# menonsamir/spiral

Hardware: AMD Instinct MI355X
Metric: server ms/query + DB GB/s vs HBM roofline, 2^20 x 256B (lower is better)
Workload: dtype u32 residues, 32x32->64-bit integer MAC (two 28-bit CRT primes)

## Files before the change

include/spiral_gpu.h:

```cpp
#ifndef SPIRAL_GPU_H
#define SPIRAL_GPU_H

#include <stddef.h>
#include <stdint.h>

#ifdef __cplusplus
extern "C" {
#endif

#define SPIRAL_GPU_ABI_VERSION 1

typedef struct spiral_gpu_params {
    uint32_t nu1;
    uint32_t nu2;
    uint32_t t_gsw;
    uint32_t t_conv;
    uint32_t t_exp;
    uint32_t t_exp_right;
    uint32_t qprime_bits;
    uint32_t direct_upload;
    uint64_t p_db;
} spiral_gpu_params;

typedef struct spiral_gpu_shape {
    uint32_t dim0, num_per, ell, m2, g, stopround;
    uint32_t n_left;
    uint32_t n_right;
    uint32_t n_query_cts;
    uint32_t n_bits;
    uint64_t qprime;
} spiral_gpu_shape;

typedef struct spiral_gpu_server spiral_gpu_server;

int spiral_gpu_abi_version(void);
const char *spiral_gpu_last_error(void);
int spiral_gpu_device_count(void);
int spiral_gpu_get_shape(const spiral_gpu_params *p, spiral_gpu_shape *out);
int spiral_gpu_has_limb_form(const spiral_gpu_params *p, uint32_t j_begin, uint32_t j_end);
int spiral_gpu_column_shard_has_limb_form(const spiral_gpu_params *p, uint32_t n_ranks);

int spiral_gpu_set_option(const char *name, int64_t value);
int spiral_gpu_get_option(const char *name, int64_t *value);

int spiral_gpu_get_tables(uint64_t *out);
int spiral_gpu_ntt_forward(uint64_t *operand, size_t npolys);
int spiral_gpu_ntt_inverse(uint64_t *operand, size_t npolys);
int spiral_gpu_to_ntt(uint64_t *out, const uint64_t *in, size_t npolys, int reduce);
int spiral_gpu_from_ntt(uint64_t *out, const uint64_t *in, size_t npolys);
int spiral_gpu_time_ntt(size_t npolys, int iters, float *fwd_ms, float *inv_ms);
int spiral_gpu_time_ntt_digits(size_t npolys, uint32_t n_digits, int iters, float *ms);
int spiral_gpu_multiply(uint64_t *out, const uint64_t *a, const uint64_t *b, size_t rs, size_t ms, size_t cs);
int spiral_gpu_add(uint64_t *out, const uint64_t *a, const uint64_t *b, size_t npolys);
int spiral_gpu_mul_by_const(uint64_t *out, const uint64_t *single_poly, const uint64_t *a, size_t npolys);
int spiral_gpu_automorph(uint64_t *out, const uint64_t *in, size_t npolys, uint64_t t);
int spiral_gpu_invert(uint64_t *out, const uint64_t *in, size_t npolys);
int spiral_gpu_gadget_invert(uint64_t *out, const uint64_t *in, size_t mx, size_t rdim, size_t cols);
int spiral_gpu_get_rescaled(uint64_t *out, const uint64_t *in, size_t n, uint64_t inp_mod, uint64_t out_mod);

size_t spiral_gpu_response_wire_bytes(const spiral_gpu_params *p, uint32_t out_n);
int spiral_gpu_response_from_wire(const spiral_gpu_params *p, uint32_t out_n, const void *wire, uint64_t *response);

int spiral_gpu_multiply_query_by_database(uint64_t *output, const uint64_t *reorientedCiphertexts,
                                          const uint64_t *database, size_t dim0, size_t num_per);
int spiral_gpu_multiply_queries_by_database(uint64_t *outputs, const uint64_t *reorientedCiphertexts, size_t n,
                                            const uint64_t *database, size_t dim0, size_t num_per);
int spiral_gpu_split_and_crt(uint64_t *out, const uint64_t *in, size_t num_per, uint32_t t_gsw);
int spiral_gpu_fold_one_further_dimension(uint64_t *cts, size_t num_per, const uint64_t *query_ct,
// ... 251 lines not shown
```

spiral_amd/_lib.py:

```python
from __future__ import annotations

import ctypes as C
import os
import subprocess

import numpy as np

HERE = os.path.dirname(os.path.abspath(__file__))
LIB_PATH = os.environ.get("SPIRAL_LIB") or os.path.join(HERE, "libspiral_gpu.so")
CSRC = os.path.join(HERE, "csrc")


class Params(C.Structure):

    _fields_ = [
        ("nu1", C.c_uint32),
        ("nu2", C.c_uint32),
        ("t_gsw", C.c_uint32),
        ("t_conv", C.c_uint32),
        ("t_exp", C.c_uint32),
        ("t_exp_right", C.c_uint32),
        ("qprime_bits", C.c_uint32),
        ("direct_upload", C.c_uint32),
        ("p_db", C.c_uint64),
# ... 14 lines not shown
        ("n_bits", C.c_uint32),
        ("qprime", C.c_uint64),
    ]


class PackShape(C.Structure):
    _fields_ = [(n, C.c_uint32) for n in ("dim0", "num_per", "ell", "g", "stopround", "n_left", "n_right", "n_query_cts", "trials")] + [
        ("qprime", C.c_uint64)
    ]


U64P = C.POINTER(C.c_uint64)

PROTOTYPES = {
    "spiral_gpu_abi_version": (C.c_int, []),
    "spiral_gpu_last_error": (C.c_char_p, []),
    "spiral_gpu_device_count": (C.c_int, []),
    "spiral_gpu_get_shape": (C.c_int, [C.POINTER(Params), C.POINTER(Shape)]),
    "spiral_gpu_has_limb_form": (C.c_int, [C.POINTER(Params), C.c_uint32, C.c_uint32]),
    "spiral_gpu_column_shard_has_limb_form": (C.c_int, [C.POINTER(Params), C.c_uint32]),
    "spiral_gpu_set_option": (C.c_int, [C.c_char_p, C.c_int64]),
    "spiral_gpu_get_option": (C.c_int, [C.c_char_p, C.POINTER(C.c_int64)]),
    "spiral_gpu_get_tables": (C.c_int, [U64P]),
    "spiral_gpu_ntt_forward": (C.c_int, [U64P, C.c_size_t]),
    "spiral_gpu_ntt_inverse": (C.c_int, [U64P, C.c_size_t]),
    "spiral_gpu_to_ntt": (C.c_int, [U64P, U64P, C.c_size_t, C.c_int]),
    "spiral_gpu_from_ntt": (C.c_int, [U64P, U64P, C.c_size_t]),
    "spiral_gpu_time_ntt": (C.c_int, [C.c_size_t, C.c_int, C.POINTER(C.c_float), C.POINTER(C.c_float)]),
    "spiral_gpu_time_ntt_digits": (C.c_int, [C.c_size_t, C.c_uint32, C.c_int, C.POINTER(C.c_float)]),
    "spiral_gpu_multiply": (C.c_int, [U64P, U64P, U64P, C.c_size_t, C.c_size_t, C.c_size_t]),
    "spiral_gpu_add": (C.c_int, [U64P, U64P, U64P, C.c_size_t]),
    "spiral_gpu_mul_by_const": (C.c_int, [U64P, U64P, U64P, C.c_size_t]),
    "spiral_gpu_automorph": (C.c_int, [U64P, U64P, C.c_size_t, C.c_uint64]),
    "spiral_gpu_invert": (C.c_int, [U64P, U64P, C.c_size_t]),
    "spiral_gpu_gadget_invert": (C.c_int, [U64P, U64P, C.c_size_t, C.c_size_t, C.c_size_t]),
    "spiral_gpu_get_rescaled": (C.c_int, [U64P, U64P, C.c_size_t, C.c_uint64, C.c_uint64]),
    "spiral_gpu_multiply_query_by_database": (C.c_int, [U64P, U64P, U64P, C.c_size_t, C.c_size_t]),
    "spiral_gpu_multiply_queries_by_database": (C.c_int, [U64P, U64P, C.c_size_t, U64P, C.c_size_t, C.c_size_t]),
    "spiral_gpu_split_and_crt": (C.c_int, [U64P, U64P, C.c_size_t, C.c_uint32]),
    "spiral_gpu_fold_one_further_dimension": (C.c_int, [U64P, C.c_size_t, U64P, U64P, C.c_uint32]),
    "spiral_gpu_expand_improved": (C.c_int, [U64P, C.c_uint32, C.c_uint32, U64P, C.c_uint32, U64P, C.c_uint32, C.c_uint32, C.c_uint32]),
    "spiral_gpu_scal_to_mat": (C.c_int, [U64P, U64P, U64P, C.c_uint32]),
    "spiral_gpu_regev_to_gsw": (C.c_int, [U64P, U64P, U64P, U64P, C.c_uint32, C.c_uint32]),
    "spiral_gpu_server_create": (C.c_int, [C.POINTER(Params), C.c_int, C.c_uint32, C.c_uint32, C.POINTER(C.c_void_p)]),
    "spiral_gpu_server_create_column_shard": (C.c_int, [C.POINTER(Params), C.c_int, C.c_uint32, C.c_uint32, C.POINTER(C.c_void_p)]),
    "spiral_gpu_server_destroy": (None, [C.c_void_p]),
# ... 265 lines not shown
```

spiral_amd/csrc/digits_device.h:

```cpp
#pragma once
#include <type_traits>

#include "common.h"
#include "ntt_device.h"

namespace spiral {

__device__ __forceinline__ uint64_t splitmix64(uint64_t x) {
    x += 0x9E3779B97F4A7C15ull;
    x = (x ^ (x >> 30)) * 0xBF58476D1CE4E5B9ull;
    x = (x ^ (x >> 27)) * 0x94D049BB133111EBull;
    return x ^ (x >> 31);
}

__device__ __forceinline__ uint64_t load_raw(const uint64_t* src, uint32_t idx, uint32_t tinv) {
    if (tinv == 0) return src[idx];
    uint32_t e = (idx * tinv) & (2 * kN - 1);
    uint64_t v = src[e & (kN - 1)];
    return (e & kN) ? kQ - v : v;
}

__device__ __forceinline__ uint64_t digit_of(uint64_t v, uint32_t k, uint32_t bits, uint64_t mask) {
    uint32_t sh = k * bits;
    if (bits <= 27u) {
        const bool up = sh >= 32u;
        const uint32_t d = __builtin_amdgcn_alignbit(up ? 0u : hi32(v), up ? hi32(v) : lo32(v), sh & 31u) & (uint32_t)mask;
        return sh >= 64 ? 0u : d;
    }
    return sh >= 64 ? 0ull : ((v >> sh) & mask);
}

__device__ __forceinline__ void udigits8(const uint64_t* raw, uint32_t k, uint32_t bits, uint32_t* d) {
    const uint32_t sh = k * bits, mask = (1u << bits) - 1u;
    if (sh >= 64u) {
#pragma unroll
        for (int r = 0; r < 8; r++) d[r] = 0;
    } else if (sh >= 32u) {
#pragma unroll
        for (int r = 0; r < 8; r++) d[r] = (hi32(raw[r]) >> (sh - 32u)) & mask;
    } else {
#pragma unroll
        for (int r = 0; r < 8; r++) d[r] = __builtin_amdgcn_alignbit(hi32(raw[r]), lo32(raw[r]), sh) & mask;
    }
}
__device__ __forceinline__ uint32_t udiv_small(uint32_t b, uint32_t d, uint32_t inv) { return d == 1u ? b : __umulhi(b, inv); }

template <bool SMALL>
__device__ __forceinline__ uint32_t digit_residue(uint32_t d, uint32_t m) {
    if constexpr (SMALL) return d;
    return d < (1u << 28) ? d : d % m;
}
constexpr uint32_t kSmallDigitBits = 27;
#define DIGIT_WIDTH_DISPATCH(bits, body) \
    do {                                 \
        if ((bits) <= kSmallDigitBits)   \
            body(std::true_type{});      \
        else                             \
            body(std::false_type{});     \
    } while (0)

struct SDigit {
    uint32_t sh_chain, sh_digit;
    uint64_t low_mask, thresh_in;
    uint64_t mask, base, thresh;
    bool has_in, may;
// ... 156 lines not shown
```

spiral_amd/csrc/kernels.h:

```cpp
#pragma once
#include <hip/hip_runtime.h>
#include <stdint.h>
#include <stdlib.h>

#include <atomic>

#include "common.h"

namespace spiral {

struct IndexMap {
    uint32_t inner, outer_stride, off;
    __host__ __device__ uint32_t operator()(uint32_t b) const { return (b / inner) * outer_stride + (b % inner) + off; }
};
inline IndexMap identity_map() { return IndexMap{1u, 1u, 0u}; }

#ifdef SPIRAL_TUNING
inline const char* tuning_env(const char* name) { return getenv(name); }
#else
inline const char* tuning_env(const char*) { return nullptr; }
#endif
struct Options {
    int fold_pair = 1, fold_chain = 1, fwd2 = -1;
    uint32_t fold_blocks = 768, sweep_mfma_min = 2, fwd2_min = 8192;
    size_t db_stage_bytes = (size_t)64 << 20;
    int one_image = 1;
    uint32_t pack_item_group = 0;
    uint32_t pack_batch_lanes = 0;
    int pack_pair_blocks = 0;
    int sweep_narrow = 0;
    uint32_t query_batch_chunk = 512;
};
Options& options();

#ifndef SPIRAL_MAX_LANES
#define SPIRAL_MAX_LANES 8
#endif
constexpr uint32_t kMaxLanes = SPIRAL_MAX_LANES;
struct Lanes {
    uint32_t n = 1;
    int64_t off[kMaxLanes] = {};
#ifdef __HIPCC__
    __device__ __forceinline__ int64_t here() const {
        const uint32_t z = blockIdx.z;
        int64_t o = 0;
#pragma unroll
        for (uint32_t q = 1; q < kMaxLanes; q++) o = z == q ? off[q] : o;
// ... 15 lines not shown
    __device__ __forceinline__ int64_t at(int64_t) const { return 0; }
#endif
};
struct Slots {
    uint32_t n = 1;
    int64_t stride = 0;
#ifdef __HIPCC__
    __device__ __forceinline__ int64_t here() const { return (int64_t)blockIdx.z * stride; }
    __device__ __forceinline__ int64_t at(int64_t s) const { return (int64_t)blockIdx.z * s; }
#endif
};
template <class P>
inline typename P::NoLanesT no_lanes(const P& p) {
    typename P::NoLanesT q{};
    static_cast<typename P::Core&>(q) = static_cast<const typename P::Core&>(p);
    return q;
}

struct DeviceTables {
    uint4* fwd = nullptr;
    uint4* inv = nullptr;
    uint64_t* neg1 = nullptr;
    uint64_t* neg1s = nullptr;
};
int tables_get(int device, DeviceTables* out);
void tables_host_rows(uint64_t* out8x2048);

constexpr bool lazy_ok(uint32_t terms) { return (unsigned __int128)terms * (2ull * kP - 1ull) * (kP - 1ull) < ((unsigned __int128)1 << 64); }
static_assert(lazy_ok(56) && lazy_ok(2 * 56) && lazy_ok(128) && !lazy_ok(129), "u64 accumulators hold up to 128 lazy products");

enum FwdLoad : uint32_t {
    LD_RAW = 0,
    LD_DIGIT = 1,
    LD_SDIGIT = 2,
    LD_LIMBS = 3,
    LD_DBGEN = 4,
    LD_PDIGIT = 6,
    LD_DBGEN1 = 7,
    LD_SDIFF = 8,
    LD_PDIFF = 9,
    LD_EXPAND = 5,
    LD_WIRE = 10,
};
constexpr uint32_t kWireCoeffBytes = 7;
constexpr uint32_t kWirePolyBytes = kWireCoeffBytes * 2048u;
enum FwdStore : uint32_t {
    ST_PK = 0,
    ST_REF = 1,
    ST_DB = 2,
// ... 422 lines not shown
```

spiral_amd/csrc/ntt.hip:

```cpp
#include <algorithm>
#include <cstdio>
#include <cstdlib>
#include <type_traits>

#include "digits_device.h"
#include "kernels.h"
#include "ntt_device.h"
#include "wire_device.h"

namespace spiral {

__device__ __forceinline__ void pk_load8_red(const uint64_t* poly, bool reduce, uint32_t tid, uint32_t* lo, uint32_t* hi) {
    uint64_t x[8];
    pk_load8(poly, tid, x);
    pk_unpack8(x, lo, hi);
    if (reduce) {
#pragma unroll
        for (int r = 0; r < 8; r++) {
            lo[r] %= kP;
            hi[r] %= kB;
        }
    }
}

// ... 411 lines not shown
    auto body = [&](auto small) {
#pragma unroll
        for (int r = 0; r < 8; r++) {
            const uint32_t d0 = (uint32_t)digit_of(raw[r], k0, bits, mask), d1 = (uint32_t)digit_of(raw[r], k1, bits, mask);
            lo0[r] = digit_residue<decltype(small)::value>(d0, kP);
            hi0[r] = digit_residue<decltype(small)::value>(d0, kB);
            lo1[r] = digit_residue<decltype(small)::value>(d1, kP);
            hi1[r] = digit_residue<decltype(small)::value>(d1, kB);
        }
    };
    DIGIT_WIDTH_DISPATCH(bits, body);
    ntt_forward_block2<false>(lo0, hi0, lo1, hi1, sh[0], sh[1], t.fwd, tid);
    const bool lazy = LOAD == LD_EXPAND || p.lazy_out != 0;
    if (!lazy) {
        canonicalize8(lo0, hi0);
        canonicalize8(lo1, hi1);
    }
    uint64_t v[8];
    pk_pack8(lo0, hi0, v);
    pk_store8(p.dst + (size_t)p.dst_map(ob + k0) * kN, tid, v);
    if (two) {
        pk_pack8(lo1, hi1, v);
        pk_store8(p.dst + (size_t)p.dst_map(ob + k1) * kN, tid, v);
    }
}

template <uint32_t STORE, bool EXPAND, class L>
__global__ __launch_bounds__(256, 8) void ntt_inverse_kernel(Tables t, InvParamsT<L> p) {
    __shared__ uint64_t sh[kLdsWords];
    const uint32_t tid = threadIdx.x, b = blockIdx.x;
    {
        const int64_t lane = p.lanes.here();
        lane_shift(p.src, lane);
        lane_shift(p.dst, lane);
        if constexpr (EXPAND) {
            lane_shift(p.cv, lane);
            lane_shift(p.query, lane);
        }
    }
    uint32_t lo[8], hi[8];
    if constexpr (EXPAND) {
        const uint32_t a = b >> 1, row = b & 1u;
        const uint32_t i = p.act.index(a, p.cnt_e);
#ifdef EXP_ABL_NO_ROW1
        if (row == 1) return;
#endif
// ... 156 lines not shown
        else                                                                                                                             \
            hipLaunchKernelGGL((KERNEL<__VA_ARGS__, NoLanes>), dim3((GRIDX), 1, 1), dim3(256), 0, s, TB, no_lanes(P));                   \
    } while (0)
#define FWD_CASE(L, S)                                                   \
    if (load == L && store == S) {                                       \
        LAUNCH_LANES(ntt_forward_kernel, nblocks, tb, p, L, S);          \
        return;                                                          \
    }

void launch_ntt_forward(const DeviceTables& t, const FwdParams& p_in, uint32_t load, uint32_t store, uint32_t nblocks, hipStream_t s) {
    if (nblocks == 0) return;
    FwdParams p = p_in;
    auto inv = [](uint32_t d) { return d > 1u ? (uint32_t)((1ull << 32) / d + 1ull) : 0u; };
    p.inv_n_digits = inv(p.n_digits);
    p.inv_te = inv(p.t_e);
    p.inv_to = inv(p.t_o);
    Tables tb{t.fwd, t.inv};
    const int fwd2_opt = options().fwd2;
    const bool fwd2 = (fwd2_opt >= 0 ? fwd2_opt != 0 : (uint64_t)nblocks * p.lanes.n >= options().fwd2_min) && p.tinv == 0;
    if ((uint64_t)nblocks * std::max({p.n_digits, p.t_e, p.t_o, 1u}) >= (1ull << 32)) {
        fprintf(stderr, "launch_ntt_forward: %u jobs exceed the range of the job-index division\n", nblocks);
        abort();
    }
    if (fwd2 && store == ST_PK && load == LD_DIGIT && p.n_digits >= 2) {
        const uint32_t nsrc = nblocks / p.n_digits;
        LAUNCH_LANES(ntt_forward2_kernel, nsrc * ((p.n_digits + 1u) / 2u), tb, p, LD_DIGIT);
        return;
    }
    if (fwd2 && store == ST_PK && load == LD_SDIFF && p.n_digits >= 2) {
        const uint32_t nsrc = nblocks / p.n_digits;
        LAUNCH_LANES(ntt_forward2_kernel, nsrc * ((p.n_digits + 1u) / 2u), tb, p, LD_SDIFF);
        return;
    }
    if (fwd2 && store == ST_PK && load == LD_PDIFF && p.n_digits >= 2) {
        const uint32_t nsrc = nblocks / p.n_digits;
        LAUNCH_LANES(ntt_forward2_kernel, nsrc * ((p.n_digits + 1u) / 2u), tb, p, LD_PDIFF);
        return;
    }
    if (fwd2 && store == ST_PK && load == LD_EXPAND) {
        const uint32_t cnt_o = p.t_o ? (nblocks - p.cnt_e * p.t_e) / p.t_o : 0u;
        LAUNCH_LANES(ntt_forward2_kernel, p.cnt_e * ((p.t_e + 1u) / 2u) + cnt_o * ((p.t_o + 1u) / 2u), tb, p, LD_EXPAND);
        return;
    }
    FWD_CASE(LD_RAW, ST_PK)
    FWD_CASE(LD_RAW, ST_REF)
    FWD_CASE(LD_DIGIT, ST_PK)
// ... 51 lines not shown
```

spiral_amd/csrc/ntt_device.h:

```cpp
#pragma once
#include "common.h"
#ifndef TWI
#define TWI(i) (i)
#endif
struct TwTable {
    __amdgpu_buffer_rsrc_t rs;
    __device__ __forceinline__ explicit TwTable(const uint4* tw) : rs(__builtin_amdgcn_make_buffer_rsrc(const_cast<uint4*>(tw), 0, 2048 * 16, 0x00020000)) {}
    __device__ __forceinline__ uint4 operator[](uint32_t i) const {
        typedef unsigned int u32x4_t __attribute__((ext_vector_type(4)));
        const u32x4_t v = __builtin_amdgcn_raw_buffer_load_b128(rs, i * 16u, 0, 0);
        return make_uint4(v.x, v.y, v.z, v.w);
    }
};
#ifdef NTT_PRIO
#define NTT_PRIO_HI() __builtin_amdgcn_s_setprio(NTT_PRIO)
#define NTT_PRIO_LO() __builtin_amdgcn_s_setprio(0)
#else
#define NTT_PRIO_HI() ((void)0)
#define NTT_PRIO_LO() ((void)0)
#endif
#ifdef NTT_ABLATE_BARRIER
#define NTT_SYNC() ((void)0)
#else
#define NTT_SYNC() __syncthreads()
// ... 216 lines not shown
        else
            dst[q * 256] = x;
    }
}
__device__ __forceinline__ void pk_unpack8(const uint64_t (&v)[8], uint32_t* lo, uint32_t* hi) {
#pragma unroll
    for (int k = 0; k < 8; k++) {
        lo[k] = lo32(v[k]);
        hi[k] = hi32(v[k]);
    }
}
__device__ __forceinline__ void pk_pack8(const uint32_t* lo, const uint32_t* hi, uint64_t (&v)[8]) {
#pragma unroll
    for (int k = 0; k < 8; k++) v[k] = pack(lo[k], hi[k]);
}

__device__ __forceinline__ void canonicalize8(uint32_t* lo, uint32_t* hi) {
#pragma unroll
    for (int k = 0; k < 8; k++) {
        lo[k] = csub_min(lo[k], kP);
        hi[k] = csub_min(hi[k], kB);
    }
}
template <bool CANONICAL = true>
__device__ __forceinline__ void ntt_forward_block(uint32_t* lo, uint32_t* hi, uint64_t* sh, const uint4* tw, uint32_t tid) {
    const TwTable tb(tw);
    Tw7 wb = tw_load8(tb, 8 + (tid >> 5), 16 + 2 * (tid >> 5), 32 + 4 * (tid >> 5));
#ifndef NTT_ABLATE_AB
    ct_radix8(lo, hi, tw, 1, 2, 4);
#endif
    NTT_PRIO_HI();
    lds_put<ix_a>(sh, tid, lo, hi);
    NTT_SYNC();
    lds_get<ix_b>(sh, tid, lo, hi);
    Tw7 wc = tw_load8(tb, 64 + (tid >> 2), 128 + 2 * (tid >> 2), 256 + 4 * (tid >> 2));
    NTT_PRIO_LO();
#ifndef NTT_ABLATE_AB
    ct_radix8_pre(lo, hi, wb);
#endif
    NTT_PRIO_HI();
    lds_put<ix_b>(sh, tid, lo, hi);
    NTT_SYNC();
    lds_get<ix_c>(sh, tid, lo, hi);
    Tw7 wd = tw_load4x2(tb, 512 + 2 * tid, 1024 + 4 * tid);
    NTT_PRIO_LO();
#pragma unroll
    for (int k = 0; k < 4; k++) {
        lo[k] = lazy_reduce(lo[k], kP);
        hi[k] = lazy_reduce(hi[k], kB);
    }
    ct_radix8_pre(lo, hi, wc);
    NTT_PRIO_HI();
#ifndef NTT_ABLATE_QUAD_EXCHANGE
    lds_put<ix_c>(sh, tid, lo, hi);
    NTT_SYNC();
    lds_get<ix_d>(sh, tid, lo, hi);
#endif
    NTT_PRIO_LO();
    ct_radix4x2_pre(lo, hi, wd);
#pragma unroll
    for (int k = 0; k < 8; k++) {
        lo[k] = lazy_reduce(lo[k], kP);
        hi[k] = lazy_reduce(hi[k], kB);
        if constexpr (CANONICAL) {
            lo[k] = csub_min(lo[k], kP);
            hi[k] = csub_min(hi[k], kB);
        }
    }
}

template <bool CANONICAL = true>
__device__ __forceinline__ void ntt_inverse_block(uint32_t* lo, uint32_t* hi, uint64_t* sh, const uint4* tw, uint32_t tid) {
    const TwTable tb(tw);
    Tw7 wd = tw_load4x2(tb, 512 + 2 * tid, 1024 + 4 * tid);
    Tw7 wc = tw_load8(tb, 64 + (tid >> 2), 128 + 2 * (tid >> 2), 256 + 4 * (tid >> 2));
    gs_radix4x2_pre(lo, hi, wd);
    NTT_PRIO_HI();
#ifndef NTT_ABLATE_QUAD_EXCHANGE
    lds_put<ix_d>(sh, tid, lo, hi);
    __syncthreads();
    lds_get<ix_c>(sh, tid, lo, hi);
#endif
    Tw7 wb = tw_load8(tb, 8 + (tid >> 5), 16 + 2 * (tid >> 5), 32 + 4 * (tid >> 5));
    NTT_PRIO_LO();
    gs_radix8_pre(lo, hi, wc);
    NTT_PRIO_HI();
    lds_put<ix_c>(sh, tid, lo, hi);
    __syncthreads();
    lds_get<ix_b>(sh, tid, lo, hi);
// ... 86 lines not shown
```

spiral_amd/csrc/primitives.cpp:

```cpp
#include "server_state.h"

thread_local std::string spiral::host::g_err;
std::atomic<uint64_t> spiral::host::g_pack_lane_batches{0};
std::atomic<uint64_t> spiral::g_mfma_sweeps{0};
std::atomic<uint64_t> spiral::host::g_db_export_ns{0};

spiral::Options& spiral::options() {
    static Options o = [] {
        Options v;
        if (const char* e = getenv("SPIRAL_FOLD_PAIR")) v.fold_pair = atoi(e) != 0;
        if (const char* e = getenv("SPIRAL_SWEEP_MFMA")) v.sweep_mfma_min = (uint32_t)strtoul(e, nullptr, 10);
        if (const char* e = getenv("SPIRAL_DB_STAGE_BYTES")) v.db_stage_bytes = (size_t)strtoull(e, nullptr, 10);
        return v;
    }();
    return o;
}

namespace {
size_t base_message_bytes(const spiral_gpu_params* p, MessageLayout (*layout)(const spiral_gpu_params&, const spiral_gpu_shape&), Form form) {
    spiral_gpu_shape s;
    return shape_of(p, &s) ? 0 : message_bytes(layout(*p, s), form);
}
}

extern "C" {

int spiral_gpu_abi_version(void) { return SPIRAL_GPU_ABI_VERSION; }

int spiral_gpu_set_option(const char* name, int64_t value) {
    if (!name) return fail("null option name");
    Options& o = options();
    const std::string n = name;
    if (n == "fold_pair") o.fold_pair = value != 0;
    else if (n == "fold_chain") o.fold_chain = value != 0;
    else if (n == "fold_blocks" && value >= 0) o.fold_blocks = (uint32_t)value;
    else if (n == "sweep_mfma_min" && value >= 0) o.sweep_mfma_min = (uint32_t)value;
    else if (n == "one_image") o.one_image = value != 0;
    else if (n == "fwd2" && value >= -1 && value <= 1) o.fwd2 = (int)value;
    else if (n == "fwd2_min" && value >= 0) o.fwd2_min = (uint32_t)value;
    else if (n == "db_stage_bytes" && value > 0) o.db_stage_bytes = (size_t)value;
    else if (n == "pack_item_group" && value >= 0 && value <= 0xFFFFFFFFll) o.pack_item_group = (uint32_t)value;
    else if (n == "pack_batch_lanes" && value >= 0 && value <= (int64_t)kMaxLanes) o.pack_batch_lanes = (uint32_t)value;
    else if (n == "pack_pair_blocks" && (value == 0 || value == 1)) o.pack_pair_blocks = (int)value;
    else if (n == "sweep_narrow" && (value == 0 || value == 1)) o.sweep_narrow = (int)value;
    else if (n == "query_batch_chunk" && value >= 1 && value <= 0xFFFFFFFFll) o.query_batch_chunk = (uint32_t)value;
    else return fail("unknown option '%s' or value %lld out of range", name, (long long)value);
    return 0;
}
int spiral_gpu_get_option(const char* name, int64_t* value) {
    if (!name || !value) return fail("null argument");
    const Options& o = options();
    const std::string n = name;
    if (n == "fold_pair") *value = o.fold_pair;
    else if (n == "fold_chain") *value = o.fold_chain;
    else if (n == "fold_blocks") *value = o.fold_blocks;
    else if (n == "sweep_mfma_min") *value = o.sweep_mfma_min;
    else if (n == "one_image") *value = o.one_image;
    else if (n == "fwd2") *value = o.fwd2;
    else if (n == "fwd2_min") *value = o.fwd2_min;
    else if (n == "db_stage_bytes") *value = (int64_t)o.db_stage_bytes;
    else if (n == "pack_item_group") *value = o.pack_item_group;
    else if (n == "pack_batch_lanes") *value = o.pack_batch_lanes;
    else if (n == "pack_pair_blocks") *value = o.pack_pair_blocks;
    else if (n == "sweep_narrow") *value = o.sweep_narrow;
    else if (n == "query_batch_chunk") *value = o.query_batch_chunk;
    else if (n == "graph_captures") *value = (int64_t)g_captures.load();
    else if (n == "pack_lane_batches") *value = (int64_t)g_pack_lane_batches.load();
    else if (n == "key_binds") *value = (int64_t)g_key_binds.load();
    else if (n == "db_export_ns") *value = (int64_t)g_db_export_ns.load();
    else if (n == "mfma_sweeps") *value = (int64_t)g_mfma_sweeps.load(std::memory_order_relaxed);
    else return fail("unknown option '%s'", name);
    return 0;
}
const char* spiral_gpu_last_error(void) { return g_err.c_str(); }
int spiral_gpu_device_count(void) {
    int n = 0;
    if (hipGetDeviceCount(&n) != hipSuccess) return 0;
    return n;
}
int spiral_gpu_get_shape(const spiral_gpu_params* p, spiral_gpu_shape* out) { return shape_of(p, out); }
int spiral_gpu_has_limb_form(const spiral_gpu_params* p, uint32_t j_begin, uint32_t j_end) {
    if (!p) return fail("null argument");
    spiral_gpu_shape s;
    spiral_gpu_params q = *p;
    q.direct_upload = 1;
    if (shape_of(&q, &s)) return -1;
    if (j_end == 0 && j_begin == 0) j_end = s.dim0;
    if (j_begin >= j_end || j_end > s.dim0) return fail("bad first-dimension shard [%u, %u) of %u", j_begin, j_end, s.dim0);
    return DbLayout::base(s.num_per, j_end - j_begin).limbs_ok() ? 1 : 0;
}
int spiral_gpu_column_shard_has_limb_form(const spiral_gpu_params* p, uint32_t n_ranks) {
    if (!p) return fail("null argument");
    spiral_gpu_shape s;
    spiral_gpu_params q = *p;
    q.direct_upload = 1;
    if (shape_of(&q, &s)) return -1;
    const uint32_t L = column_shard_columns(s.num_per, 0, n_ranks);
    if (!L) return 0;
    return DbLayout::base(L, s.dim0).limbs_ok() ? 1 : 0;
}
int spiral_gpu_get_tables(uint64_t* out) {
    if (!out) return fail("null argument");
    tables_host_rows(out);
    return 0;
}

int spiral_gpu_ntt_forward(uint64_t* operand, size_t npolys) {
    DeviceTables tb;
    if (current_tables(&tb)) return -1;
    Scratch sc;
    uint64_t* d = sc.upload(operand, npolys * kRefNtt);
    if (!d) return fail("device allocation/upload failed");
    FwdParams fp{};
    fp.src = d;
    fp.dst = d;
    fp.src_map = fp.dst_map = identity_map();
    fp.n_digits = 1;
    launch_ntt_forward(tb, fp, LD_LIMBS, ST_REF, (uint32_t)npolys, 0);
    HIP_OK(hipMemcpy(operand, d, npolys * kRefNtt * sizeof(uint64_t), hipMemcpyDeviceToHost));
    return 0;
}

int spiral_gpu_ntt_inverse(uint64_t* operand, size_t npolys) {
    DeviceTables tb;
    if (current_tables(&tb)) return -1;
    Scratch sc;
// ... 395 lines not shown
```

spiral_amd/csrc/tables.cpp:

```cpp
#include <mutex>
#include <vector>

#include "common.h"
#include "kernels.h"
#include "transform_jobs.h"

namespace spiral {

static uint64_t powmod(uint64_t b, uint64_t e, uint64_t m) {
    unsigned __int128 r = 1, x = b % m;
    while (e) {
        if (e & 1) r = r * x % m;
        x = x * x % m;
        e >>= 1;
    }
    return (uint64_t)r;
}
static uint32_t bitrev11(uint32_t x) {
    uint32_t r = 0;
    for (uint32_t i = 0; i < kLogN; i++) r |= ((x >> i) & 1u) << (kLogN - 1 - i);
    return r;
}

void tables_host_rows(uint64_t* out) {
    const uint64_t mods[2] = {kP, kB}, psis[2] = {66687, 158221};
    for (int n = 0; n < 2; n++) {
        uint64_t m = mods[n], psi = psis[n], ipsi = powmod(psi, 2 * kN - 1, m);
        uint64_t f = 1, v = (m + 1) / 2;
        for (uint32_t i = 0; i < kN; i++) {
            uint32_t k = bitrev11(i);
            out[(4 + 2 * n) * kN + k] = f;
            out[(5 + 2 * n) * kN + k] = (f << 32) / m;
            out[(0 + 2 * n) * kN + k] = v;
            out[(1 + 2 * n) * kN + k] = (v << 32) / m;
            f = (uint64_t)((unsigned __int128)f * psi % m);
            v = (uint64_t)((unsigned __int128)v * ipsi % m);
        }
    }
}

static std::mutex g_mu;
static DeviceTables g_tables[16];
static bool g_ready[16];

int tables_get(int device, DeviceTables* out) {
    if (device < 0 || device >= 16) return -1;
    std::lock_guard<std::mutex> lk(g_mu);
    if (!g_ready[device]) {
        std::vector<uint64_t> rows(8 * kN);
        tables_host_rows(rows.data());
        std::vector<uint4> fwd(kN), inv(kN);
        for (uint32_t i = 0; i < kN; i++) {
            fwd[i] = make_uint4((uint32_t)rows[4 * kN + i], (uint32_t)rows[5 * kN + i], (uint32_t)rows[6 * kN + i], (uint32_t)rows[7 * kN + i]);
        }
        {
            const uint64_t mods[2] = {kP, kB};
            uint32_t w[2][kN];
            for (int n = 0; n < 2; n++) {
                const uint64_t m = mods[n], ninv = powmod(kN, m - 2, m);
                for (uint32_t i = 0; i < kN; i++) w[n][i] = (uint32_t)(rows[(0 + 2 * n) * kN + i] * 2 % m);
                w[n][1] = (uint32_t)((unsigned __int128)w[n][1] * ninv % m);
                w[n][0] = (uint32_t)ninv;
            }
            for (uint32_t i = 0; i < kN; i++)
                inv[i] = make_uint4(w[0][i], (uint32_t)(((uint64_t)w[0][i] << 32) / kP), w[1][i], (uint32_t)(((uint64_t)w[1][i] << 32) / kB));
        }
        DeviceTables t;
        if (hipSetDevice(device) != hipSuccess) return -1;
        if (hipMalloc(&t.fwd, kN * sizeof(uint4)) != hipSuccess) return -1;
        if (hipMalloc(&t.inv, kN * sizeof(uint4)) != hipSuccess) return -1;
        if (hipMalloc(&t.neg1, (size_t)kLogN * kN * sizeof(uint64_t)) != hipSuccess) return -1;
        if (hipMemcpy(t.fwd, fwd.data(), kN * sizeof(uint4), hipMemcpyHostToDevice) != hipSuccess) return -1;
        if (hipMemcpy(t.inv, inv.data(), kN * sizeof(uint4), hipMemcpyHostToDevice) != hipSuccess) return -1;
        std::vector<uint64_t> raw((size_t)kLogN * kN, 0);
        for (uint32_t r = 0; r < kLogN; r++) raw[(size_t)r * kN + (kN - (1u << r))] = kQ - 1;
        uint64_t* d_raw = nullptr;
        if (hipMalloc(&d_raw, raw.size() * sizeof(uint64_t)) != hipSuccess) return -1;
        if (hipMemcpy(d_raw, raw.data(), raw.size() * sizeof(uint64_t), hipMemcpyHostToDevice) != hipSuccess) return -1;
        host::launch_job(t, host::raw_job(d_raw, t.neg1, kLogN), 0);
        if (hipDeviceSynchronize() != hipSuccess) return -1;
        (void)hipFree(d_raw);
        std::vector<uint64_t> w((size_t)kLogN * kN);
        if (hipMemcpy(w.data(), t.neg1, w.size() * sizeof(uint64_t), hipMemcpyDeviceToHost) != hipSuccess) return -1;
        for (uint64_t& x : w) x = (((x & 0xffffffffull) << 32) / kP) | ((((x >> 32) << 32) / kB) << 32);
        if (hipMalloc(&t.neg1s, w.size() * sizeof(uint64_t)) != hipSuccess) return -1;
        if (hipMemcpy(t.neg1s, w.data(), w.size() * sizeof(uint64_t), hipMemcpyHostToDevice) != hipSuccess) return -1;
        g_tables[device] = t;
        g_ready[device] = true;
    }
    *out = g_tables[device];
    return 0;
}

}
```

spiral_amd/ops.py:

```python
from __future__ import annotations

import ctypes as C

import numpy as np

from ._lib import SEED_BYTES, SEED_PACK_PUB_PARAMS, SEED_PACK_QUERY, SEED_PUB_PARAMS, SEED_QUERY, WIRE_POLY_BYTES, U64P, Params, Shape, check, lib, wire_bytes

N = 2048
P = 268369921
B = 249561089
Q = P * B

__all__ = [
    "N", "P", "B", "Q", "make_params", "get_shape", "has_limb_form", "column_shard_has_limb_form", "get_tables", "ntt_forward", "ntt_inverse", "to_ntt", "to_ntt_no_reduce", "from_ntt",
    "multiply", "add", "mul_by_const", "automorph", "invert", "gadget_invert", "getRescaled", "multiplyQueryByDatabase", "multiplyQueriesByDatabase", "split_and_crt",
    "foldOneFurtherDimension", "expandImproved", "scalToMat", "regevToGSW", "time_ntt", "time_ntt_digits", "response_wire_bytes", "response_from_wire",
    "query_wire_bytes", "pub_params_wire_bytes", "pack_query_wire_bytes", "pack_pub_params_wire_bytes", "raw_to_wire", "raw_from_wire",
    "query_seeded_bytes", "pub_params_seeded_bytes", "pack_query_seeded_bytes", "pack_pub_params_seeded_bytes", "seed_expand",
    "SEED_BYTES", "SEED_QUERY", "SEED_PUB_PARAMS", "SEED_PACK_QUERY", "SEED_PACK_PUB_PARAMS",
    "set_option", "get_option", "options",
]


def _p(a: np.ndarray):
    assert a.dtype == np.uint64 and a.flags["C_CONTIGUOUS"]
    return a.ctypes.data_as(U64P)


def _c(a) -> np.ndarray:
    return np.ascontiguousarray(a, dtype=np.uint64)


def set_option(name: str, value: int) -> None:
    check(lib().spiral_gpu_set_option(name.encode(), int(value)))


def get_option(name: str) -> int:
# ... 29 lines not shown
    return s


def has_limb_form(p: Params, j_begin: int = 0, j_end: int = 0) -> bool:
    rc = lib().spiral_gpu_has_limb_form(C.byref(p), j_begin, j_end)
    if rc < 0:
        check(rc)
    return bool(rc)


def column_shard_has_limb_form(p: Params, n_ranks: int) -> bool:
    rc = lib().spiral_gpu_column_shard_has_limb_form(C.byref(p), n_ranks)
    if rc < 0:
        check(rc)
    return bool(rc)


def get_tables() -> np.ndarray:
    out = np.zeros((8, N), dtype=np.uint64)
    check(lib().spiral_gpu_get_tables(_p(out)))
    return out


def ntt_forward(operand) -> np.ndarray:
    x = _c(operand).copy()
    check(lib().spiral_gpu_ntt_forward(_p(x), x.size // (2 * N)))
    return x


def ntt_inverse(operand) -> np.ndarray:
    x = _c(operand).copy()
    check(lib().spiral_gpu_ntt_inverse(_p(x), x.size // (2 * N)))
    return x


def to_ntt(raw) -> np.ndarray:
    raw = _c(raw)
    out = np.zeros(raw.shape[:-1] + (2, N), dtype=np.uint64)
    check(lib().spiral_gpu_to_ntt(_p(out), _p(raw), raw.size // N, 1))
    return out


def to_ntt_no_reduce(raw) -> np.ndarray:
    raw = _c(raw)
    out = np.zeros(raw.shape[:-1] + (2, N), dtype=np.uint64)
    check(lib().spiral_gpu_to_ntt(_p(out), _p(raw), raw.size // N, 0))
# ... 190 lines not shown
```

Measured before the change: 0.7312.

## Compute first six forward-NTT stages of small gadget digits with int8 MFMA

Adds an MFMA-based forward NTT kernel for gadget-decomposed digits of at most 8 bits. The first six butterfly stages are precomputed as a 64x64 matrix per CRT modulus, split into signed byte limbs, and applied to byte-packed digit panels with i8 matrix instructions. Partial sums are recombined with a Shoup-style reduction before the remaining stages run with the existing radix code. One raw load is reused for a group of digits, which cuts repeated source reads and scalar butterfly work. The cost is extra LDS panels, more registers for the operands, and a new path with tricky correctness. It is enabled by default above a size threshold.

After: 0.7312, median of 4. About the same (+0.0%).

```diff
diff --git a/include/spiral_gpu.h b/include/spiral_gpu.h
--- a/include/spiral_gpu.h
+++ b/include/spiral_gpu.h
@@ -44,6 +44,7 @@
 int spiral_gpu_get_option(const char *name, int64_t *value);
 
 int spiral_gpu_get_tables(uint64_t *out);
+int spiral_gpu_get_digit_matrix(uint32_t *m, uint32_t *operands);
 int spiral_gpu_ntt_forward(uint64_t *operand, size_t npolys);
 int spiral_gpu_ntt_inverse(uint64_t *operand, size_t npolys);
 int spiral_gpu_to_ntt(uint64_t *out, const uint64_t *in, size_t npolys, int reduce);
diff --git a/spiral_amd/_lib.py b/spiral_amd/_lib.py
--- a/spiral_amd/_lib.py
+++ b/spiral_amd/_lib.py
@@ -60,6 +60,7 @@
     "spiral_gpu_set_option": (C.c_int, [C.c_char_p, C.c_int64]),
     "spiral_gpu_get_option": (C.c_int, [C.c_char_p, C.POINTER(C.c_int64)]),
     "spiral_gpu_get_tables": (C.c_int, [U64P]),
+    "spiral_gpu_get_digit_matrix": (C.c_int, [C.c_void_p, C.c_void_p]),
     "spiral_gpu_ntt_forward": (C.c_int, [U64P, C.c_size_t]),
     "spiral_gpu_ntt_inverse": (C.c_int, [U64P, C.c_size_t]),
     "spiral_gpu_to_ntt": (C.c_int, [U64P, U64P, C.c_size_t, C.c_int]),
diff --git a/spiral_amd/csrc/digits_device.h b/spiral_amd/csrc/digits_device.h
--- a/spiral_amd/csrc/digits_device.h
+++ b/spiral_amd/csrc/digits_device.h
@@ -41,6 +41,32 @@
     } else {
 #pragma unroll
         for (int r = 0; r < 8; r++) d[r] = __builtin_amdgcn_alignbit(hi32(raw[r]), lo32(raw[r]), sh) & mask;
+    }
+}
+__device__ __forceinline__ uint32_t mx_bytes4(uint32_t x0, uint32_t x1, uint32_t x2, uint32_t x3, uint32_t b) {
+    const uint32_t sel = ((4u + b) << 8) | b;
+    return __builtin_amdgcn_perm(__builtin_amdgcn_perm(x3, x2, sel), __builtin_amdgcn_perm(x1, x0, sel), 0x05040100u);
+}
+__device__ __forceinline__ void mx_digit_words(const uint64_t* raw, uint32_t k, uint32_t bits, uint32_t (&w)[2]) {
+    if ((8u % bits) == 0) {
+        const uint32_t o = k * bits, B = o >> 3;
+        if (B < 4u) {
+            w[0] = mx_bytes4(lo32(raw[0]), lo32(raw[1]), lo32(raw[2]), lo32(raw[3]), B);
+            w[1] = mx_bytes4(lo32(raw[4]), lo32(raw[5]), lo32(raw[6]), lo32(raw[7]), B);
+        } else if (B < 8u) {
+            w[0] = mx_bytes4(hi32(raw[0]), hi32(raw[1]), hi32(raw[2]), hi32(raw[3]), B - 4u);
+            w[1] = mx_bytes4(hi32(raw[4]), hi32(raw[5]), hi32(raw[6]), hi32(raw[7]), B - 4u);
+        } else {
+            w[0] = w[1] = 0u;
+        }
+        const uint32_t mask = ((1u << bits) - 1u) * 0x01010101u;
+        w[0] = ((w[0] >> (o & 7u)) & mask) ^ 0x80808080u;
+        w[1] = ((w[1] >> (o & 7u)) & mask) ^ 0x80808080u;
+    } else {
+        uint32_t d[8];
+        udigits8(raw, k, bits, d);
+        w[0] = (d[0] | (d[1] << 8) | (d[2] << 16) | (d[3] << 24)) ^ 0x80808080u;
+        w[1] = (d[4] | (d[5] << 8) | (d[6] << 16) | (d[7] << 24)) ^ 0x80808080u;
     }
 }
 __device__ __forceinline__ uint32_t udiv_small(uint32_t b, uint32_t d, uint32_t inv) { return d == 1u ? b : __umulhi(b, inv); }
diff --git a/spiral_amd/csrc/kernels.h b/spiral_amd/csrc/kernels.h
--- a/spiral_amd/csrc/kernels.h
+++ b/spiral_amd/csrc/kernels.h
@@ -22,7 +22,8 @@
 #endif
 struct Options {
     int fold_pair = 1, fold_chain = 1, fwd2 = -1;
-    uint32_t fold_blocks = 768, sweep_mfma_min = 2, fwd2_min = 8192;
+    int fwd_mx = -1;
+    uint32_t fold_blocks = 768, sweep_mfma_min = 2, fwd2_min = 8192, fwd_mx_min = 8192;
     size_t db_stage_bytes = (size_t)64 << 20;
     int one_image = 1;
     uint32_t pack_item_group = 0;
@@ -84,9 +85,14 @@
     uint4* inv = nullptr;
     uint64_t* neg1 = nullptr;
     uint64_t* neg1s = nullptr;
-};
+    uint4* mx = nullptr;
+};
+constexpr uint32_t kMxLimbU4 = 2 * 4 * 4 * 64;
+constexpr uint32_t kMxTableU4 = kMxLimbU4 + 2 * 4 * 64;
 int tables_get(int device, DeviceTables* out);
 void tables_host_rows(uint64_t* out8x2048);
+void digit_mx_matrix(uint32_t* M2x64x64);
+void digit_mx_operands(uint32_t* out);
 
 constexpr bool lazy_ok(uint32_t terms) { return (unsigned __int128)terms * (2ull * kP - 1ull) * (kP - 1ull) < ((unsigned __int128)1 << 64); }
 static_assert(lazy_ok(56) && lazy_ok(2 * 56) && lazy_ok(128) && !lazy_ok(129), "u64 accumulators hold up to 128 lazy products");
diff --git a/spiral_amd/csrc/ntt.hip b/spiral_amd/csrc/ntt.hip
--- a/spiral_amd/csrc/ntt.hip
+++ b/spiral_amd/csrc/ntt.hip
@@ -457,6 +457,104 @@
     if (two) {
         pk_pack8(lo1, hi1, v);
         pk_store8(p.dst + (size_t)p.dst_map(ob + k1) * kN, tid, v);
+    }
+}
+
+template <uint32_t LOAD, class L>
+__global__ __launch_bounds__(256, 3) void ntt_forward_mx_kernel(Tables t, const uint4* __restrict__ mx, FwdParamsT<L> p) {
+    static_assert(LOAD == LD_EXPAND || LOAD == LD_DIGIT || LOAD == LD_PDIGIT, "unsigned digit loaders only");
+    __shared__ uint64_t sh[kLdsWords];
+    __shared__ __attribute__((aligned(16))) uint8_t panel[2][kMxPanelBytes];
+    const uint32_t tid = threadIdx.x, lane = tid & 63u, wv = tid >> 6, b = blockIdx.x;
+    {
+        const int64_t lane_off = p.lanes.here();
+        lane_shift(p.src, lane_off);
+        lane_shift(p.dst, lane_off);
+    }
+    uint32_t tdim, gi, s, bits;
+    const uint64_t* src;
+    if constexpr (LOAD == LD_EXPAND) {
+        const uint32_t ge = (p.t_e + kMxGroup - 1u) / kMxGroup, go = (p.t_o + kMxGroup - 1u) / kMxGroup, je = p.cnt_e * ge;
+        uint32_t a;
+        if (b < je) {
+            tdim = p.t_e;
+            a = b / ge;
+            gi = b - a * ge;
+            s = a * tdim;
+        } else {
+            tdim = p.t_o;
+            const uint32_t bb = b - je;
+            a = bb / go;
+            gi = bb - a * go;
+            s = p.cnt_e * p.t_e + a * tdim;
+            a += p.cnt_e;
+        }
+        src = p.src + (size_t)a * 2u * kN;
+        bits = get_bits_per(tdim);
+    } else {
+        tdim = p.n_digits;
+        const uint32_t gp = (tdim + kMxGroup - 1u) / kMxGroup;
+        s = b / gp;
+        gi = b - s * gp;
+        bits = p.bits;
+        if constexpr (LOAD == LD_DIGIT) {
+            src = p.src + (size_t)p.src_map(s) * kN;
+        } else {
+            uint32_t sp;
+            if (p.pmode == PM_GSW) {
+                sp = s;
+            } else if (p.pmode == PM_FOLD) {
+                const uint32_t per_t = 4u * p.fold_np, tr = s / per_t, rem = s - tr * per_t;
+                sp = (tr * p.pk_num_per + (rem >> 1)) * 2u + (rem & 1u);
+            } else {
+                sp = s * p.pk_num_per * 2u;
+            }
+            src = p.src + (size_t)sp * kN;
+        }
+    }
+    uint64_t raw[8];
+#pragma unroll
+    for (int r = 0; r < 8; r++) raw[r] = src[ix_a(tid, r)];
+    const MxOperands op = mx_load(mx, wv, lane);
+    const TwTable tb(t.fwd);
+    auto dst_of = [&](uint32_t k) -> uint32_t {
+        if constexpr (LOAD == LD_EXPAND) {
+            return p.dst_map(s + k);
+        } else if constexpr (LOAD == LD_DIGIT) {
+            return p.dst_map(s * tdim + k);
+        } else {
+            if (p.pmode == PM_GSW) return (s >> 1) * (2u * tdim) + 2u * k + (s & 1u);
+            if (p.pmode == PM_FOLD) {
+                const uint32_t per_t = 4u * p.fold_np, tr = s / per_t, rem = s - tr * per_t, ip = rem >> 1, row = rem & 1u;
+                const uint32_t hh = ip / p.fold_np, i = ip - hh * p.fold_np;
+                return ((tr * p.fold_np + i) * 2u + hh) * (2u * tdim) + 2u * k + row;
+            }
+            return s * tdim + k;
+        }
+    };
+    const bool lazy = LOAD == LD_EXPAND || p.lazy_out != 0;
+    const uint32_t k0 = gi * kMxGroup, k1 = min(k0 + kMxGroup, tdim);
+    uint32_t dw[2];
+    mx_digit_words(raw, k0, bits, dw);
+    mx_panel_put(panel[0], tid, dw);
+    for (uint32_t k = k0; k < k1; k++) {
+        const uint32_t pb = (k - k0) & 1u;
+        __syncthreads();
+        const Tw7 wc = tw_load8(tb, 64 + (tid >> 2), 128 + 2 * (tid >> 2), 256 + 4 * (tid >> 2));
+        mx_first_six(panel[pb], op, wv, lane, sh);
+        if (k + 1u < k1) {
+            mx_digit_words(raw, k + 1u, bits, dw);
+            mx_panel_put(panel[pb ^ 1u], tid, dw);
+        }
+        __syncthreads();
+        uint32_t lo[8], hi[8];
+        lds_get<ix_c>(sh, tid, lo, hi);
+        const Tw7 wd = tw_load4x2(tb, 512 + 2 * tid, 1024 + 4 * tid);
+        ntt_forward_cd<false>(lo, hi, sh, wc, wd, tid);
+        if (!lazy) canonicalize8(lo, hi);
+        uint64_t v[8];
+        pk_pack8(lo, hi, v);
+        pk_store8(p.dst + (size_t)dst_of(k) * kN, tid, v);
     }
 }
 
@@ -659,6 +757,25 @@
         fprintf(stderr, "launch_ntt_forward: %u jobs exceed the range of the job-index division\n", nblocks);
         abort();
     }
+    const int mx_opt = options().fwd_mx;
+    const bool mx_on = (mx_opt >= 0 ? mx_opt != 0 : (uint64_t)nblocks * p.lanes.n >= options().fwd_mx_min) && p.tinv == 0 && store == ST_PK;
+    auto mx_groups = [](uint32_t t) { return (t + kMxGroup - 1u) / kMxGroup; };
+#define LAUNCH_MX(LOADK, GRIDX)                                                                                                                        \
+    do {                                                                                                                                               \
+        if (p.lanes.n > 1)                                                                                                                             \
+            hipLaunchKernelGGL((ntt_forward_mx_kernel<LOADK, Lanes>), dim3((GRIDX), 1, p.lanes.n), dim3(256), 0, s, tb, t.mx, p);                      \
+        else                                                                                                                                           \
+            hipLaunchKernelGGL((ntt_forward_mx_kernel<LOADK, NoLanes>), dim3((GRIDX), 1, 1), dim3(256), 0, s, tb, t.mx, no_lanes(p));                  \
+        return;                                                                                                                                        \
+    } while (0)
+    if (mx_on && load == LD_EXPAND) {
+        const uint32_t cnt_o = p.t_o ? (nblocks - p.cnt_e * p.t_e) / p.t_o : 0u;
+        if ((p.cnt_e == 0 || get_bits_per(p.t_e) <= kMxDigitBits) && (cnt_o == 0 || get_bits_per(p.t_o) <= kMxDigitBits))
+            LAUNCH_MX(LD_EXPAND, p.cnt_e * mx_groups(p.t_e) + cnt_o * mx_groups(p.t_o));
+    }
+    if (mx_on && load == LD_DIGIT && p.bits <= kMxDigitBits) LAUNCH_MX(LD_DIGIT, (nblocks / p.n_digits) * mx_groups(p.n_digits));
+    if (mx_on && load == LD_PDIGIT && p.bits <= kMxDigitBits) LAUNCH_MX(LD_PDIGIT, (nblocks / p.n_digits) * mx_groups(p.n_digits));
+#undef LAUNCH_MX
     if (fwd2 && store == ST_PK && load == LD_DIGIT && p.n_digits >= 2) {
         const uint32_t nsrc = nblocks / p.n_digits;
         LAUNCH_LANES(ntt_forward2_kernel, nsrc * ((p.n_digits + 1u) / 2u), tb, p, LD_DIGIT);
diff --git a/spiral_amd/csrc/ntt_device.h b/spiral_amd/csrc/ntt_device.h
--- a/spiral_amd/csrc/ntt_device.h
+++ b/spiral_amd/csrc/ntt_device.h
@@ -262,6 +262,32 @@
         hi[k] = csub_min(hi[k], kB);
     }
 }
+template <bool CANONICAL>
+__device__ __forceinline__ void ntt_forward_cd(uint32_t* lo, uint32_t* hi, uint64_t* sh, const Tw7& wc, const Tw7& wd, uint32_t tid) {
+#pragma unroll
+    for (int k = 0; k < 4; k++) {
+        lo[k] = lazy_reduce(lo[k], kP);
+        hi[k] = lazy_reduce(hi[k], kB);
+    }
+    ct_radix8_pre(lo, hi, wc);
+    NTT_PRIO_HI();
+#ifndef NTT_ABLATE_QUAD_EXCHANGE
+    lds_put<ix_c>(sh, tid, lo, hi);
+    NTT_SYNC();
+    lds_get<ix_d>(sh, tid, lo, hi);
+#endif
+    NTT_PRIO_LO();
+    ct_radix4x2_pre(lo, hi, wd);
+#pragma unroll
+    for (int k = 0; k < 8; k++) {
+        lo[k] = lazy_reduce(lo[k], kP);
+        hi[k] = lazy_reduce(hi[k], kB);
+        if constexpr (CANONICAL) {
+            lo[k] = csub_min(lo[k], kP);
+            hi[k] = csub_min(hi[k], kB);
+        }
+    }
+}
 template <bool CANONICAL = true>
 __device__ __forceinline__ void ntt_forward_block(uint32_t* lo, uint32_t* hi, uint64_t* sh, const uint4* tw, uint32_t tid) {
     const TwTable tb(tw);
@@ -284,27 +310,59 @@
     lds_get<ix_c>(sh, tid, lo, hi);
     Tw7 wd = tw_load4x2(tb, 512 + 2 * tid, 1024 + 4 * tid);
     NTT_PRIO_LO();
-#pragma unroll
-    for (int k = 0; k < 4; k++) {
-        lo[k] = lazy_reduce(lo[k], kP);
-        hi[k] = lazy_reduce(hi[k], kB);
-    }
-    ct_radix8_pre(lo, hi, wc);
-    NTT_PRIO_HI();
-#ifndef NTT_ABLATE_QUAD_EXCHANGE
-    lds_put<ix_c>(sh, tid, lo, hi);
-    NTT_SYNC();
-    lds_get<ix_d>(sh, tid, lo, hi);
-#endif
-    NTT_PRIO_LO();
-    ct_radix4x2_pre(lo, hi, wd);
-#pragma unroll
-    for (int k = 0; k < 8; k++) {
-        lo[k] = lazy_reduce(lo[k], kP);
-        hi[k] = lazy_reduce(hi[k], kB);
-        if constexpr (CANONICAL) {
-            lo[k] = csub_min(lo[k], kP);
-            hi[k] = csub_min(hi[k], kB);
+    ntt_forward_cd<CANONICAL>(lo, hi, sh, wc, wd, tid);
+}
+
+typedef int mx_v4i __attribute__((ext_vector_type(4)));
+constexpr uint32_t kMxDigitBits = 8;
+constexpr uint32_t kMxGroup = 8;
+constexpr uint32_t kMxPanelStride = 80;
+constexpr uint32_t kMxPanelBytes = 32 * kMxPanelStride;
+constexpr uint32_t kMxShoup16P = (uint32_t)((1ull << 48) / kP), kMxShoup16B = (uint32_t)((1ull << 48) / kB);
+struct MxOperands {
+    mx_v4i a[2][4];
+    mx_v4i c0[2];
+};
+__device__ __forceinline__ MxOperands mx_load(const uint4* mx, uint32_t wv, uint32_t lane) {
+    MxOperands op;
+#pragma unroll
+    for (uint32_t pr = 0; pr < 2; pr++) {
+#pragma unroll
+        for (uint32_t i = 0; i < 4; i++) {
+            const uint4 v = mx[((pr * 4u + i) * 4u + wv) * 64u + lane];
+            op.a[pr][i] = mx_v4i{(int)v.x, (int)v.y, (int)v.z, (int)v.w};
+        }
+        const uint4 c = mx[2u * 4u * 4u * 64u + (pr * 4u + wv) * 64u + lane];
+        op.c0[pr] = mx_v4i{(int)c.x, (int)c.y, (int)c.z, (int)c.w};
+    }
+    return op;
+}
+__device__ __forceinline__ void mx_panel_put(uint8_t* panel, uint32_t tid, const uint32_t (&w)[2]) {
+    *reinterpret_cast<uint2*>(panel + (tid & 31u) * kMxPanelStride + (tid >> 5) * 8u) = make_uint2(w[0], w[1]);
+}
+__device__ __forceinline__ uint32_t mx_recombine(int s0, int s1, int s2, int s3, uint32_t ws16, uint32_t m) {
+    const uint32_t low = ((uint32_t)s1 << 8) + (uint32_t)s0, high = ((uint32_t)s3 << 8) + (uint32_t)s2;
+    return low + ((high << 16) - __umulhi(high, ws16) * m);
+}
+__device__ __forceinline__ void mx_first_six(const uint8_t* panel, const MxOperands& op, uint32_t wv, uint32_t lane, uint64_t* sh) {
+    const mx_v4i zero = {0, 0, 0, 0}, mp = {(int)kP, (int)kP, (int)kP, (int)kP}, mb = {(int)kB, (int)kB, (int)kB, (int)kB};
+#pragma unroll
+    for (uint32_t t = 0; t < 2; t++) {
+        const uint4 bv = *reinterpret_cast<const uint4*>(panel + (16u * t + (lane & 15u)) * kMxPanelStride + (lane >> 4) * 16u);
+        const mx_v4i b = {(int)bv.x, (int)bv.y, (int)bv.z, (int)bv.w};
+        mx_v4i s[2][4];
+#pragma unroll
+        for (int pr = 0; pr < 2; pr++) {
+            s[pr][0] = __builtin_amdgcn_mfma_i32_16x16x64_i8(op.a[pr][0], b, op.c0[pr], 0, 0, 0);
+            s[pr][1] = __builtin_amdgcn_mfma_i32_16x16x64_i8(op.a[pr][1], b, zero, 0, 0, 0);
+            s[pr][2] = __builtin_amdgcn_mfma_i32_16x16x64_i8(op.a[pr][2], b, pr ? mb : mp, 0, 0, 0);
+            s[pr][3] = __builtin_amdgcn_mfma_i32_16x16x64_i8(op.a[pr][3], b, zero, 0, 0, 0);
+        }
+#pragma unroll
+        for (uint32_t e = 0; e < 4; e++) {
+            const uint32_t row = 16u * wv + 4u * (lane >> 4) + e;
+            sh[lds_ix(32u * row + 16u * t + (lane & 15u))] = pack(mx_recombine(s[0][0][e], s[0][1][e], s[0][2][e], s[0][3][e], kMxShoup16P, kP),
+                                                                  mx_recombine(s[1][0][e], s[1][1][e], s[1][2][e], s[1][3][e], kMxShoup16B, kB));
         }
     }
 }
diff --git a/spiral_amd/csrc/primitives.cpp b/spiral_amd/csrc/primitives.cpp
--- a/spiral_amd/csrc/primitives.cpp
+++ b/spiral_amd/csrc/primitives.cpp
@@ -38,6 +38,8 @@
     else if (n == "one_image") o.one_image = value != 0;
     else if (n == "fwd2" && value >= -1 && value <= 1) o.fwd2 = (int)value;
     else if (n == "fwd2_min" && value >= 0) o.fwd2_min = (uint32_t)value;
+    else if (n == "fwd_mx" && value >= -1 && value <= 1) o.fwd_mx = (int)value;
+    else if (n == "fwd_mx_min" && value >= 0 && value <= 0xFFFFFFFFll) o.fwd_mx_min = (uint32_t)value;
     else if (n == "db_stage_bytes" && value > 0) o.db_stage_bytes = (size_t)value;
     else if (n == "pack_item_group" && value >= 0 && value <= 0xFFFFFFFFll) o.pack_item_group = (uint32_t)value;
     else if (n == "pack_batch_lanes" && value >= 0 && value <= (int64_t)kMaxLanes) o.pack_batch_lanes = (uint32_t)value;
@@ -58,6 +60,8 @@
     else if (n == "one_image") *value = o.one_image;
     else if (n == "fwd2") *value = o.fwd2;
     else if (n == "fwd2_min") *value = o.fwd2_min;
+    else if (n == "fwd_mx") *value = o.fwd_mx;
+    else if (n == "fwd_mx_min") *value = o.fwd_mx_min;
     else if (n == "db_stage_bytes") *value = (int64_t)o.db_stage_bytes;
     else if (n == "pack_item_group") *value = o.pack_item_group;
     else if (n == "pack_batch_lanes") *value = o.pack_batch_lanes;
@@ -102,6 +106,12 @@
 int spiral_gpu_get_tables(uint64_t* out) {
     if (!out) return fail("null argument");
     tables_host_rows(out);
+    return 0;
+}
+int spiral_gpu_get_digit_matrix(uint32_t* m, uint32_t* operands) {
+    if (!m && !operands) return fail("null argument");
+    if (m) digit_mx_matrix(m);
+    if (operands) digit_mx_operands(operands);
     return 0;
 }
 
diff --git a/spiral_amd/csrc/tables.cpp b/spiral_amd/csrc/tables.cpp
--- a/spiral_amd/csrc/tables.cpp
+++ b/spiral_amd/csrc/tables.cpp
@@ -39,6 +39,53 @@
     }
 }
 
+void digit_mx_matrix(uint32_t* M) {
+    std::vector<uint64_t> rows(8 * kN);
+    tables_host_rows(rows.data());
+    const uint64_t mods[2] = {kP, kB};
+    for (int n = 0; n < 2; n++) {
+        const uint64_t m = mods[n], *W = rows.data() + (size_t)(4 + 2 * n) * kN;
+        for (uint32_t i = 0; i < 64; i++) {
+            uint64_t v[64] = {};
+            v[i] = 1;
+            for (uint32_t s = 0; s < 6; s++) {
+                const uint32_t nb = 1u << s, half = 32u >> s;
+                for (uint32_t b = 0; b < nb; b++)
+                    for (uint32_t t = 0; t < half; t++) {
+                        uint64_t &x = v[b * 2 * half + t], &y = v[b * 2 * half + t + half];
+                        const uint64_t T = W[nb + b] * y % m, x0 = x;
+                        x = (x0 + T) % m;
+                        y = (x0 + m - T) % m;
+                    }
+            }
+            for (uint32_t o = 0; o < 64; o++) M[((size_t)n * 64 + o) * 64 + i] = (uint32_t)v[o];
+        }
+    }
+}
+void digit_mx_operands(uint32_t* out) {
+    std::vector<uint32_t> M(2 * 64 * 64);
+    digit_mx_matrix(M.data());
+    const uint32_t mods[2] = {kP, kB};
+    uint8_t* bytes = reinterpret_cast<uint8_t*>(out);
+    for (uint32_t pr = 0; pr < 2; pr++)
+        for (uint32_t wv = 0; wv < 4; wv++)
+            for (uint32_t lane = 0; lane < 64; lane++) {
+                for (uint32_t i = 0; i < 4; i++)
+                    for (uint32_t b = 0; b < 16; b++) {
+                        const uint32_t o = 16 * wv + (lane & 15), kap = 16 * (lane >> 4) + b, ip = (kap >> 3) + 8 * (kap & 7);
+                        const uint32_t a = M[((size_t)pr * 64 + o) * 64 + ip];
+                        const uint32_t w = (a >= (1u << 28) - 0x808080u ? a - mods[pr] : a) + 0x808080u;
+                        bytes[((((size_t)pr * 4 + i) * 4 + wv) * 64 + lane) * 16 + b] = i < 3 ? (uint8_t)(((w >> (8 * i)) & 0xFFu) ^ 0x80u) : (uint8_t)(w >> 24);
+                    }
+                for (uint32_t e = 0; e < 4; e++) {
+                    const uint32_t o = 16 * wv + 4 * (lane >> 4) + e;
+                    uint64_t sum = 0;
+                    for (uint32_t ip = 0; ip < 64; ip++) sum += M[((size_t)pr * 64 + o) * 64 + ip];
+                    out[(kMxLimbU4 + ((size_t)pr * 4 + wv) * 64 + lane) * 4 + e] = 2 * mods[pr] + (uint32_t)(128 * sum % mods[pr]);
+                }
+            }
+}
+
 static std::mutex g_mu;
 static DeviceTables g_tables[16];
 static bool g_ready[16];
@@ -72,6 +119,12 @@
         if (hipMalloc(&t.neg1, (size_t)kLogN * kN * sizeof(uint64_t)) != hipSuccess) return -1;
         if (hipMemcpy(t.fwd, fwd.data(), kN * sizeof(uint4), hipMemcpyHostToDevice) != hipSuccess) return -1;
         if (hipMemcpy(t.inv, inv.data(), kN * sizeof(uint4), hipMemcpyHostToDevice) != hipSuccess) return -1;
+        {
+            std::vector<uint32_t> mx((size_t)kMxTableU4 * 4);
+            digit_mx_operands(mx.data());
+            if (hipMalloc(&t.mx, kMxTableU4 * sizeof(uint4)) != hipSuccess) return -1;
+            if (hipMemcpy(t.mx, mx.data(), kMxTableU4 * sizeof(uint4), hipMemcpyHostToDevice) != hipSuccess) return -1;
+        }
         std::vector<uint64_t> raw((size_t)kLogN * kN, 0);
         for (uint32_t r = 0; r < kLogN; r++) raw[(size_t)r * kN + (kN - (1u << r))] = kQ - 1;
         uint64_t* d_raw = nullptr;
diff --git a/spiral_amd/ops.py b/spiral_amd/ops.py
--- a/spiral_amd/ops.py
+++ b/spiral_amd/ops.py
@@ -12,7 +12,7 @@
 Q = P * B
 
 __all__ = [
-    "N", "P", "B", "Q", "make_params", "get_shape", "has_limb_form", "column_shard_has_limb_form", "get_tables", "ntt_forward", "ntt_inverse", "to_ntt", "to_ntt_no_reduce", "from_ntt",
+    "N", "P", "B", "Q", "make_params", "get_shape", "has_limb_form", "column_shard_has_limb_form", "get_tables", "get_digit_matrix", "ntt_forward", "ntt_inverse", "to_ntt", "to_ntt_no_reduce", "from_ntt",
     "multiply", "add", "mul_by_const", "automorph", "invert", "gadget_invert", "getRescaled", "multiplyQueryByDatabase", "multiplyQueriesByDatabase", "split_and_crt",
     "foldOneFurtherDimension", "expandImproved", "scalToMat", "regevToGSW", "time_ntt", "time_ntt_digits", "response_wire_bytes", "response_from_wire",
     "query_wire_bytes", "pub_params_wire_bytes", "pack_query_wire_bytes", "pack_pub_params_wire_bytes", "raw_to_wire", "raw_from_wire",
@@ -88,6 +88,12 @@
     return out
 
 
+def get_digit_matrix():
+    m, ops = np.zeros((2, 64, 64), dtype=np.uint32), np.zeros(10240, dtype=np.uint32)
+    check(lib().spiral_gpu_get_digit_matrix(m.ctypes.data, ops.ctypes.data))
+    return m, ops
+
+
 def ntt_forward(operand) -> np.ndarray:
     x = _c(operand).copy()
     check(lib().spiral_gpu_ntt_forward(_p(x), x.size // (2 * N)))
```
